# ClimeTrend/DMD-ERA5

Measured on AMD Instinct MI355X. Metric: rank-r SVD GB/s on ERA5 snapshot matrix (X resident in HBM), higher is better.
Workload: dtype f32; 1 GPU; cfg2: 1038240x8760 fp32 synthetic low-rank(64)+noise, row-centred, rank-50 method-of-snapshots SVD; m_per_gpu=1038240, m_total=1038240, n=8760, rank=50, svd_type=standard

## Files before the change

dmd_era5_amd/csrc/gemm_tn.hip:

```cpp
#include <stdarg.h>
#include <stdio.h>
#include <stdlib.h>

#include <algorithm>
#include <vector>

#include "dmdx_common.h"

thread_local unsigned long long* dmdx_clock_probe_ptr = nullptr;

int dmdx_device_cus() {
  static int cached[64] = {0};
  int dev = 0;
  if (hipGetDevice(&dev) != hipSuccess || dev < 0 || dev >= 64) return -1;
  if (cached[dev] == 0) {
    int v = 0;
    cached[dev] = (hipDeviceGetAttribute(&v, hipDeviceAttributeMultiprocessorCount, dev) == hipSuccess && v > 0) ? v : -1;
  }
  return cached[dev];
}

namespace {

constexpr int BT = 128;
constexpr int BK = 32;
constexpr int FOLD = 128;
constexpr int NTH = 256;

struct TnParams {
  const float* A;
  const float* B;
  int64_t lda, ldb;
  int64_t K;
  int nrow, ncol;
  int ntr, ntc;
  int ntiles;
  int syrk;
  int nsplit;
  int chunks_total;
  int chunks_per_split;
  double* P;
};

constexpr int MAXB = 16;
struct TnBatch {
  const float* A[MAXB];
  const float* B[MAXB];
  int64_t lda[MAXB];
  int64_t ldb[MAXB];
  int64_t K[MAXB];
  int chunks_total[MAXB];
  int chunks_per_split[MAXB];
  int nsplit[MAXB];
  int unit_begin[MAXB + 1];
  int slab_begin[MAXB + 1];
  int nblocks;
  unsigned long long* clk;
};

constexpr int SR = 8;
__device__ __host__ inline void decode_tri(int t, int nt, int& ta, int& tb) {
  int r0 = 0;
  for (;;) {
    int nrows = nt - r0 < SR ? nt - r0 : SR;
    int ncols = nt - r0;
    int cnt = nrows * (nrows + 1) / 2 + (ncols - nrows) * nrows;
    if (t < cnt) break;
    t -= cnt;
    r0 += SR;
  }
  int nrows = nt - r0 < SR ? nt - r0 : SR;
  int head = nrows * (nrows + 1) / 2;
  if (t < head) {
    int c = 0;
    while (t >= c + 1) { t -= c + 1; ++c; }
    tb = r0 + c;
    ta = r0 + t;
  } else {
    t -= head;
    tb = r0 + nrows + t / nrows;
    ta = r0 + t % nrows;
  }
}

__device__ inline void decode_tile(int syrk, int ntr, int ntc, int t, int& ta, int& tb) {
  if (syrk) {
    decode_tri(t, ntr, ta, tb);
  } else {
    int per_sr = SR * ntc;
    int sr = t / per_sr;
    int r0 = sr * SR;
    int nrows = ntr - r0 < SR ? ntr - r0 : SR;
    int tt = t - sr * per_sr;
    tb = tt / nrows;
    ta = r0 + tt % nrows;
  }
}

__device__ __forceinline__ int swz(int col) { return (col >> 1) & 7; }

__device__ inline f32x4 load4_tail(const float* p, int64_t k, int64_t kend) {
  f32x4 v = {0.f, 0.f, 0.f, 0.f};
#pragma unroll
  for (int e = 0; e < 4; ++e)
    if (k + e < kend) v[e] = p[e];
  return v;
}

#ifdef DMDX_STAMPS
__device__ unsigned long long dmdx_stamp[12];
#define DMDX_STAMP(var)                                                        \
  do {                                                                         \
    __builtin_amdgcn_sched_barrier(0);                                         \
    asm volatile("s_memtime %0\n\ts_waitcnt lgkmcnt(0)" : "=s"(var)::"memory"); \
    __builtin_amdgcn_sched_barrier(0);                                         \
  } while (0)
#else
#define DMDX_STAMP(var) do { } while (0)
#endif

#define DMDX_LDS_PTR(p) ((__attribute__((address_space(3))) void*)(p))
#define DMDX_GLB_PTR(p) ((const __attribute__((address_space(1))) void*)(p))

template <bool DMA, int ABL, int SK, int H16 = 0>
__device__ __forceinline__ void tn_unit(const TnParams& p, const int split, const int row0, const int col0,
                                        double* Pt, float* lds) {
  static_assert(!H16 || SK >= 1, "a 16-row block only below at least one 32-row block");
#ifdef DMDX_STAMPS
  unsigned long long pt0;
  asm volatile("s_memtime %0\n\ts_waitcnt lgkmcnt(0)" : "=s"(pt0)::"memory");
#endif
  constexpr int TM = SK ? 32 * SK + 16 * H16 : BT;
  constexpr int MI = SK ? SK : 2;
  constexpr int NI = SK ? 1 : 2;
  constexpr int NPA = (TM + 31) / 32;
  constexpr int NPIECE = TM / 8;
  constexpr int OPA = TM * BK, OPB = BT * BK, STG = OPA + OPB;

  const int c_begin = split * p.chunks_per_split;
  int c_end = c_begin + p.chunks_per_split;
  if (c_end > p.chunks_total) c_end = p.chunks_total;
  const int nchunks = c_end - c_begin;
  const int64_t kend = p.K;
  const int tail_chunk = (kend % BK) ? p.chunks_total - 1 : -1;

  const int tid = threadIdx.x;
  const int lane = tid & 63;
  const int wave = __builtin_amdgcn_readfirstlane(tid >> 6);
  const int wr = SK ? 0 : wave >> 1, wc = SK ? wave : wave & 1;
  const int l31 = lane & 31, lh = lane >> 5;

  const int ra0 = row0 < p.nrow ? row0 : p.nrow - 1;
  const int cb0 = col0 < p.ncol ? col0 : p.ncol - 1;
  const float* Abase = p.A + (int64_t)ra0 * p.lda;
  const float* Bbase = p.B + (int64_t)cb0 * p.ldb;
  unsigned aoff[NPA], boff[4];
  int stsa[NPA], stsb[4];
  int kqa[NPA], kqb[4];
#pragma unroll
  for (int i = 0; i < 4; ++i) {
    const int lc = DMA ? 32 * wave + 8 * i + (lane >> 3) : (tid >> 3) + 32 * i;
    const int q = DMA ? ((lane & 7) ^ swz(lc)) : (tid & 7);
    int cb = col0 + lc;
    cb = cb < p.ncol ? cb : p.ncol - 1;
    boff[i] = (unsigned)((int64_t)(cb - cb0) * p.ldb + 4 * q);
    stsb[i] = lc * BK + 4 * (DMA ? (lane & 7) : ((tid & 7) ^ swz(lc)));
    kqb[i] = 4 * q;
  }
#pragma unroll
  for (int i = 0; i < NPA; ++i) {
    const int lc = DMA ? (H16 ? 8 * (wave + 4 * i) : (TM / 4) * wave + 8 * i) + (lane >> 3) : (tid >> 3) + 32 * i;
    const int q = DMA ? ((lane & 7) ^ swz(lc)) : (tid & 7);
    int ca = row0 + (lc < TM ? lc : TM - 1);
    ca = ca < p.nrow ? ca : p.nrow - 1;
    aoff[i] = (unsigned)((int64_t)(ca - ra0) * p.lda + 4 * q);
    stsa[i] = lc * BK + 4 * (DMA ? (lane & 7) : ((tid & 7) ^ swz(lc)));
    kqa[i] = 4 * q;
  }

  const char* Adma = reinterpret_cast<const char*>(Abase) - (H16 ? 0 : 3072);
  const char* Bdma = reinterpret_cast<const char*>(Bbase) - 3072;
  unsigned aoffb[NPA], boffb[4];
#pragma unroll
  for (int i = 0; i < 4; ++i) boffb[i] = 4u * boff[i] + 3072u - 1024u * i;
#pragma unroll
  for (int i = 0; i < NPA; ++i) aoffb[i] = H16 ? 4u * aoff[i] : 4u * aoff[i] + 3072u - 1024u * i;

  f32x16 acc[MI][NI];
#pragma unroll
  for (int mi = 0; mi < MI; ++mi)
#pragma unroll
    for (int ni = 0; ni < NI; ++ni)
#pragma unroll
      for (int r = 0; r < 16; ++r) acc[mi][ni][r] = 0.f;

  f32x16 acc2[MI][NI];
#pragma unroll
  for (int mi = 0; mi < MI; ++mi)
#pragma unroll
    for (int ni = 0; ni < NI; ++ni)
#pragma unroll
      for (int r = 0; r < 16; ++r) acc2[mi][ni][r] = 0.f;
  f32x4 acch[2] = {{0.f, 0.f, 0.f, 0.f}, {0.f, 0.f, 0.f, 0.f}}, acch2[2] = {{0.f, 0.f, 0.f, 0.f}, {0.f, 0.f, 0.f, 0.f}};
  const int l15 = lane & 15, lkk = lane >> 4;
  const int lane_off = (64 * wr + 4 * lh) * BT + (SK ? 32 : 64) * wc + l31;
#define DMDX_BLOCK_OFF(mi, ni, r) ((32 * (mi) + ((r) & 3) + 8 * ((r) >> 2)) * BT + 32 * (ni))
#define DMDX_FOLD(mi, ni)                                                         \
  do {                                                                            \
    acc2[mi][ni] += acc[mi][ni];                                                  \
    _Pragma("unroll") for (int r = 0; r < 16; ++r) acc[mi][ni][r] = 0.f;          \
  } while (0)
#define DMDX_COMMIT(mi, ni)                                                       \
  do {                                                                            \
    double* q_ = Pt + lane_off;                                                   \
    _Pragma("unroll") for (int r = 0; r < 16; ++r)                                \
        __builtin_nontemporal_store((double)(acc[mi][ni][r] + acc2[mi][ni][r]),   \
                                    q_ + DMDX_BLOCK_OFF(mi, ni, r));              \
  } while (0)
#define DMDX_COMMIT_H16()                                                         \
  do {                                                                            \
    _Pragma("unroll") for (int hh = 0; hh < 2; ++hh)                              \
        _Pragma("unroll") for (int r = 0; r < 4; ++r)                             \
            __builtin_nontemporal_store((double)(acch[hh][r] + acch2[hh][r]),     \
                                        Pt + (32 * SK + 4 * lkk + r) * BT + 32 * wc + 16 * hh + l15); \
  } while (0)
#define DMDX_COMMIT_ALL()                                                         \
  do {                                                                            \
    if constexpr (H16 != 0) DMDX_COMMIT_H16();                                    \
    DMDX_COMMIT(0, 0);                                                            \
    if constexpr (MI >= 2) DMDX_COMMIT(MI >= 2 ? 1 : 0, 0);                       \
    if constexpr (NI == 2) {                                                      \
      DMDX_COMMIT(0, NI - 1);                                                     \
      DMDX_COMMIT(1, NI - 1);                                                     \
    }                                                                             \
    if constexpr (MI == 3) DMDX_COMMIT(MI - 1, 0);                                \
  } while (0)

  if (nchunks <= 0) {
    DMDX_COMMIT_ALL();
    return;
  }

  auto stage_regs = [&](int chunk, int st, bool tail) {
    const int64_t k0 = (int64_t)chunk * BK;
    f32x4 ra[NPA], rb[4];
#pragma unroll
    for (int i = 0; i < 4; ++i) {
      const float* pb = Bbase + k0 + boff[i];
      rb[i] = tail ? load4_tail(pb, k0 + kqb[i], kend) : f32x4{pb[0], pb[1], pb[2], pb[3]};
    }
#pragma unroll
    for (int i = 0; i < NPA; ++i) {
      const float* pa = Abase + k0 + aoff[i];
      ra[i] = tail ? load4_tail(pa, k0 + kqa[i], kend) : f32x4{pa[0], pa[1], pa[2], pa[3]};
    }
    const bool a_last_ok = !H16 || (DMA ? wave + 4 * (NPA - 1) < NPIECE : (tid >> 3) + 32 * (NPA - 1) < TM);
    float* as = lds + st * STG;
    float* bs = lds + st * STG + OPA;
#pragma unroll
    for (int i = 0; i < 4; ++i) *reinterpret_cast<f32x4*>(bs + stsb[i]) = rb[i];
#pragma unroll
    for (int i = 0; i < NPA; ++i)
      if (i + 1 < NPA || a_last_ok) *reinterpret_cast<f32x4*>(as + stsa[i]) = ra[i];
  };
#define DMDX_DMA_OP4(ptr, la, o0, o1, o2, o3)                                                      \
  asm volatile("s_mov_b32 m0, %[la_]\n\ts_nop 0\n\t"                                               \
               "global_load_lds_dwordx4 %[a0], %[ap_]\n\t"                                         \
               "global_load_lds_dwordx4 %[a1], %[ap_] offset:1024\n\t"                             \
               "global_load_lds_dwordx4 %[a2], %[ap_] offset:2048\n\t"                             \
               "global_load_lds_dwordx4 %[a3], %[ap_] offset:3072"                                 \
               :: [la_] "s"(la), [ap_] "s"(ptr), [a0] "v"(o0), [a1] "v"(o1), [a2] "v"(o2), [a3] "v"(o3) \
               : "memory")
#define DMDX_DMA_OP3(ptr, la, o0, o1, o2)                                                          \
  asm volatile("s_mov_b32 m0, %[la_]\n\ts_nop 0\n\t"                                               \
               "global_load_lds_dwordx4 %[a0], %[ap_]\n\t"                                         \
               "global_load_lds_dwordx4 %[a1], %[ap_] offset:1024\n\t"                             \
               "global_load_lds_dwordx4 %[a2], %[ap_] offset:2048"                                 \
               :: [la_] "s"(la), [ap_] "s"(ptr), [a0] "v"(o0), [a1] "v"(o1), [a2] "v"(o2)           \
               : "memory")
#define DMDX_DMA_OP1(ptr, la, o0)                                                                  \
  asm volatile("s_mov_b32 m0, %[la_]\n\ts_nop 0\n\t"                                               \
               "global_load_lds_dwordx4 %[a0], %[ap_]"                                             \
               :: [la_] "s"(la), [ap_] "s"(ptr), [a0] "v"(o0)                                       \
               : "memory")
#define DMDX_DMA_OP2(ptr, la, o0, o1)                                                              \
  asm volatile("s_mov_b32 m0, %[la_]\n\ts_nop 0\n\t"                                               \
               "global_load_lds_dwordx4 %[a0], %[ap_]\n\t"                                         \
               "global_load_lds_dwordx4 %[a1], %[ap_] offset:1024"                                 \
               :: [la_] "s"(la), [ap_] "s"(ptr), [a0] "v"(o0), [a1] "v"(o1)                         \
               : "memory")
#define DMDX_DMA_A(ap, la)                                                                         \
  do {                                                                                             \
    if constexpr (H16 != 0) {                                                                      \
      _Pragma("unroll") for (int i_ = 0; i_ < NPA; ++i_)                                           \
          if (i_ + 1 < NPA || wave + 4 * (NPA - 1) < NPIECE) DMDX_DMA_OP1(ap, (la) + 4096u * i_, aoffb[i_]); \
    } else if constexpr (NPA == 4) DMDX_DMA_OP4(ap, la, aoffb[0], aoffb[1], aoffb[NPA - 2], aoffb[NPA - 1]); \
    else if constexpr (NPA == 3) DMDX_DMA_OP3(ap, la, aoffb[0], aoffb[1], aoffb[NPA - 1]);         \
    else if constexpr (NPA == 2) DMDX_DMA_OP2(ap, la, aoffb[0], aoffb[NPA - 1]);                   \
    else DMDX_DMA_OP1(ap, la, aoffb[0]);                                                           \
  } while (0)
#define DMDX_DMA_B(bp, lb) DMDX_DMA_OP4(bp, lb, boffb[0], boffb[1], boffb[2], boffb[3])
#define DMDX_DMA_NEXT(ap, bp, la, lb) \
  do {                                \
    DMDX_DMA_A(ap, la);               \
    DMDX_DMA_B(bp, lb);               \
  } while (0)
  auto stage_dma = [&](int chunk, int st) {
    const int64_t k0 = (int64_t)chunk * BK;
    float* as = lds + st * STG + (H16 ? 8 * wave : (TM / 4) * wave) * BK;
    float* bs = lds + st * STG + OPA + (32 * wave) * BK;
    DMDX_DMA_NEXT(Adma + 4 * k0, Bdma + 4 * k0, (unsigned)(uintptr_t)DMDX_LDS_PTR(as),
                  (unsigned)(uintptr_t)DMDX_LDS_PTR(bs));
  };
  auto stage = [&](int chunk, int st) {
    if (DMA) {
      if (chunk != tail_chunk) stage_dma(chunk, st);
      else stage_regs(chunk, st, true);
    } else {
      stage_regs(chunk, st, chunk == tail_chunk);
    }
  };

  f32x4 fa0[MI], fb0[NI], fa1[MI], fb1[NI];
  f32x4 hA[2] = {{0.f, 0.f, 0.f, 0.f}, {0.f, 0.f, 0.f, 0.f}};
  f32x4 hB[2][2] = {{{0.f, 0.f, 0.f, 0.f}, {0.f, 0.f, 0.f, 0.f}}, {{0.f, 0.f, 0.f, 0.f}, {0.f, 0.f, 0.f, 0.f}}};
  int foff[4], foffh[2];
#pragma unroll
  for (int t = 0; t < 4; ++t) {
    foff[t] = l31 * BK + 4 * ((2 * t + lh) ^ swz(l31));
    if (t < 2) foffh[t] = l15 * BK + 4 * ((4 * t + lkk) ^ swz(l15));
  }
  const int frag_a = 64 * wr * BK, frag_b = (SK ? 32 : 64) * wc * BK;
#define DMDX_READ_FRAGS(FA, FB, st, t)                                               \
  do {                                                                               \
    if constexpr (H16 != 0) {                                                        \
      if constexpr ((t) % 2 == 0) {                                                  \
        const float* ah_ = lds + (st) * STG + 32 * SK * BK + foffh[(t) / 2];         \
        const float* bh_ = lds + (st) * STG + OPA + frag_b + foffh[(t) / 2];         \
        hA[(t) / 2] = *reinterpret_cast<const f32x4*>(ah_);                          \
        hB[(t) / 2][0] = *reinterpret_cast<const f32x4*>(bh_);                       \
        hB[(t) / 2][1] = *reinterpret_cast<const f32x4*>(bh_ + 16 * BK);             \
      }                                                                              \
    }                                                                                \
    const float* as_ = lds + (st) * STG + frag_a + foff[t];                          \
    const float* bs_ = lds + (st) * STG + OPA + frag_b + foff[t];                    \
    FA[0] = *reinterpret_cast<const f32x4*>(as_);                                    \
    if constexpr (MI >= 2) FA[MI >= 2 ? 1 : 0] = *reinterpret_cast<const f32x4*>(as_ + 32 * BK); \
    if constexpr (MI == 3) FA[MI - 1] = *reinterpret_cast<const f32x4*>(as_ + 64 * BK); \
    FB[0] = *reinterpret_cast<const f32x4*>(bs_);                                    \
    if constexpr (NI == 2) FB[NI - 1] = *reinterpret_cast<const f32x4*>(bs_ + 32 * BK); \
  } while (0)

  stage(c_begin, 0);
  if (nchunks > 1 && !(ABL & 1)) stage(c_begin + 1, 1);
  if (DMA) __builtin_amdgcn_s_waitcnt(0x0f70);
  __syncthreads();
  DMDX_READ_FRAGS(fa0, fb0, 0, 0);

#define DMDX_MFMA4(FA, FB, j)                                                                   \
  do {                                                                                          \
    _Pragma("unroll") for (int mi_ = 0; mi_ < MI; ++mi_)                                        \
        _Pragma("unroll") for (int ni_ = 0; ni_ < NI; ++ni_) acc[mi_][ni_] =                    \
            __builtin_amdgcn_mfma_f32_32x32x2f32(FA[mi_][j], FB[ni_][j], acc[mi_][ni_], 0, 0, 0); \
  } while (0)
#define DMDX_KSTEP(FA, FB, i)                                      \
  do {                                                             \
    DMDX_MFMA4(FA, FB, 0);                                         \
    DMDX_MFMA4(FA, FB, 1);                                         \
    DMDX_MFMA4(FA, FB, 2);                                         \
    DMDX_MFMA4(FA, FB, 3);                                         \
    if constexpr (H16 != 0) {                                      \
      _Pragma("unroll") for (int s_ = 0; s_ < 2; ++s_)             \
          _Pragma("unroll") for (int hh_ = 0; hh_ < 2; ++hh_) acch[hh_] = \
              __builtin_amdgcn_mfma_f32_16x16x4f32(hA[(i) / 2][2 * ((i) % 2) + s_], hB[(i) / 2][hh_][2 * ((i) % 2) + s_], acch[hh_], 0, 0, 0); \
    }                                                              \
    __builtin_amdgcn_sched_group_barrier(0x008, 4 * MI * NI + 4 * H16, 0);   \
  } while (0)

#ifdef DMDX_STAMPS
  unsigned long long rt0, rt1, ct0;
  asm volatile("s_memrealtime %0\n\ts_memtime %1\n\ts_waitcnt lgkmcnt(0)" : "=s"(rt0), "=s"(ct0)::"memory");
  unsigned long long st0 = 0, st1 = 0, st2 = 0, st2b = 0, st3 = 0, st4 = 0, sa0 = 0, sa1 = 0, sa2 = 0, sa3 = 0, sa5 = 0;
#endif
  int cur = 0;
  for (int c = 0; c < nchunks; ++c) {
    DMDX_STAMP(st0);
    const bool has_next = (c + 1 < nchunks) && !(ABL & 1);
    const int phase = c & (FOLD / 4 - 1), fq = (c / (FOLD / 4)) & 3;
    DMDX_STAMP(st1);
    DMDX_READ_FRAGS(fa1, fb1, cur, 1);
    __builtin_amdgcn_sched_group_barrier(0x100, MI + NI, 0);
    DMDX_KSTEP(fa0, fb0, 0);
    DMDX_READ_FRAGS(fa0, fb0, cur, 2);
    __builtin_amdgcn_sched_group_barrier(0x100, MI + NI + 3 * H16, 0);
    DMDX_KSTEP(fa1, fb1, 1);
    DMDX_READ_FRAGS(fa1, fb1, cur, 3);
    __builtin_amdgcn_sched_group_barrier(0x100, MI + NI, 0);
    DMDX_KSTEP(fa0, fb0, 2);
    DMDX_STAMP(st2);

    if (DMA) __builtin_amdgcn_s_waitcnt(0x0f70);
    DMDX_STAMP(st2b);
    if (!(ABL & 2)) __syncthreads();
    if (c + 2 < nchunks && !(ABL & 1)) stage(c_begin + c + 2, cur);
    cur ^= 1;
    DMDX_STAMP(st3);
    if (has_next) DMDX_READ_FRAGS(fa0, fb0, cur, 0);
    __builtin_amdgcn_sched_group_barrier(0x100, MI + NI + 3 * H16, 0);
    DMDX_KSTEP(fa1, fb1, 3);
    if (!(ABL & 8) && phase == FOLD / 4 - 1) {
      switch (fq) {
        case 0: DMDX_FOLD(0, 0); break;
        case 1:
          if constexpr (NI == 2) { DMDX_FOLD(0, NI - 1); }
          else if constexpr (MI == 3) { DMDX_FOLD(MI - 1, 0); }
          break;
        case 2: if constexpr (MI >= 2) { DMDX_FOLD(MI >= 2 ? 1 : 0, 0); } break;
        default:
          if constexpr (NI == 2) { DMDX_FOLD(1, NI - 1); }
          if constexpr (H16 != 0) {
#pragma unroll
            for (int hh = 0; hh < 2; ++hh) {
              acch2[hh] += acch[hh];
              acch[hh] = f32x4{0.f, 0.f, 0.f, 0.f};
            }
          }
          break;
      }
    }
#ifdef DMDX_STAMPS
    DMDX_STAMP(st4);
    sa0 += st1 - st0; sa1 += st2 - st1; sa2 += st3 - st2b; sa3 += st4 - st3; sa5 += st2b - st2;
#endif
  }
#ifdef DMDX_STAMPS
  if (lane == 0) {
    atomicAdd(&dmdx_stamp[0], sa0); atomicAdd(&dmdx_stamp[1], sa1);
    atomicAdd(&dmdx_stamp[2], sa2); atomicAdd(&dmdx_stamp[3], sa3);
    atomicAdd(&dmdx_stamp[5], sa5);
    asm volatile("s_memrealtime %0\n\ts_waitcnt lgkmcnt(0)" : "=s"(rt1)::"memory");
    atomicAdd(&dmdx_stamp[6], st4 - ct0);
    atomicAdd(&dmdx_stamp[7], rt1 - rt0);
    atomicAdd(&dmdx_stamp[4], (unsigned long long)nchunks);
    atomicAdd(&dmdx_stamp[8], ct0 - pt0);
    atomicAdd(&dmdx_stamp[10], 1ull);
  }
#endif
  DMDX_COMMIT_ALL();
#ifdef DMDX_STAMPS
  {
    unsigned long long et1;
    asm volatile("s_waitcnt vmcnt(0)\n\ts_memtime %0\n\ts_waitcnt lgkmcnt(0)" : "=s"(et1)::"memory");
    if (lane == 0) atomicAdd(&dmdx_stamp[9], et1 - st4);
  }
#endif
#undef DMDX_READ_FRAGS
#undef DMDX_MFMA4
#undef DMDX_KSTEP
#undef DMDX_DMA_NEXT
#undef DMDX_DMA_A
#undef DMDX_DMA_B
#undef DMDX_DMA_OP4
#undef DMDX_DMA_OP2
#undef DMDX_DMA_OP1
#undef DMDX_DMA_OP3
#undef DMDX_FOLD
#undef DMDX_COMMIT_ALL
#undef DMDX_COMMIT_H16
#undef DMDX_COMMIT
#undef DMDX_BLOCK_OFF
}

__device__ __forceinline__ int xcd_unit(int b, int total) {
  const int g = b >> 9;
  return ((g << 9) + 512 <= total) ? (g << 9) + (b & 7) * 64 + ((b & 511) >> 3) : b;
}

#ifndef DMDX_TN_ABL
#define DMDX_TN_ABL 0
#endif

template <bool DMA, int SK = 0, int H16 = 0>
__global__ __launch_bounds__(NTH, 2) void syrk_batch_kernel(TnParams p, TnBatch bt) {
  constexpr int TM = SK ? 32 * SK + 16 * H16 : BT;
  __shared__ __attribute__((aligned(16))) float lds[2 * (TM + BT) * BK];
  const int b = blockIdx.x;
  int j = 0;
  while (j + 1 < bt.nblocks && b >= bt.unit_begin[j + 1]) ++j;
  const int total = bt.nsplit[j] * p.ntiles;
  const int local = b - bt.unit_begin[j];
  if (local >= total) return;
  const int pos = xcd_unit(local, total);
  const int split = pos / p.ntiles;
  const int tile = pos - split * p.ntiles;
  int ta, tb;
  decode_tile(p.syrk, p.ntr, p.ntc, tile, ta, tb);
  p.A = bt.A[j];
  p.B = bt.B[j];
  p.lda = bt.lda[j];
  p.ldb = bt.ldb[j];
  p.K = bt.K[j];
  p.chunks_total = bt.chunks_total[j];
  p.chunks_per_split = bt.chunks_per_split[j];
  double* Pt = p.P + ((size_t)(bt.slab_begin[j] + split) * p.ntiles + tile) * (TM * BT);
  unsigned long long c0 = 0, r0 = 0;
  if (bt.clk != nullptr) {
    c0 = __builtin_amdgcn_s_memtime();
    r0 = __builtin_amdgcn_s_memrealtime();
  }
  tn_unit<DMA, DMDX_TN_ABL, SK, H16>(p, split, ta * TM, tb * BT, Pt, lds);
  if (bt.clk != nullptr) {
    const unsigned long long c1 = __builtin_amdgcn_s_memtime(), r1 = __builtin_amdgcn_s_memrealtime();
    if (threadIdx.x == 0) {
      atomicAdd(&bt.clk[0], c1 - c0);
      atomicAdd(&bt.clk[1], r1 - r0);
      atomicAdd(&bt.clk[2], 1ull);
    }
  }
}

__global__ __launch_bounds__(256) void gemm_tn_reduce_kernel(
    const double* P, int nsplit, int ntiles, int ntr, int ntc, int syrk, int nrow, int ncol,
    double* D64, int64_t ld64, float* D32, int64_t ld32, int accumulate, int tm) {
  __shared__ double tr[32][33];
  const int nsb = ((tm + 31) / 32) * 4;
  const int tile = blockIdx.x / nsb;
  const int sb = blockIdx.x - tile * nsb;
  const int tile_elems = tm * BT;
  int ta, tb;
  decode_tile(syrk, ntr, ntc, tile, ta, tb);
  const int row0 = ta * tm, col0 = tb * BT;
  const int tx = threadIdx.x & 31, ty = threadIdx.x >> 5;
  const bool diag = syrk && (ta == tb);
  const int si = (sb >> 2) * 32, sj = (sb & 3) * 32;
  if (diag && si > sj) return;
  if (row0 + si >= nrow || col0 + sj >= ncol) return;
  double v[4] = {0.0, 0.0, 0.0, 0.0};
  const double* src = P + (size_t)tile * tile_elems + (si + ty) * BT + sj + tx;
  for (int sp = 0; sp < nsplit; ++sp) {
    const double* q = src + (size_t)sp * ntiles * tile_elems;
#pragma unroll
    for (int k = 0; k < 4; ++k)
      if (si + ty + 8 * k < tm) v[k] += q[8 * k * BT];
  }
#pragma unroll
  for (int k = 0; k < 4; ++k) {
    const int i = si + ty + 8 * k, j = sj + tx;
    const int gi = row0 + i, gj = col0 + j;
    const bool keep = !(diag && i > j) && i < tm;
    if (keep && gi < nrow && gj < ncol) {
      double o = v[k];
      if (accumulate) o += D64[(int64_t)gi * ld64 + gj];
      D64[(int64_t)gi * ld64 + gj] = o;
      if (D32) D32[(int64_t)gi * ld32 + gj] = (float)o;
    }
    tr[ty + 8 * k][tx] = v[k];
  }
  if (syrk) {
    __syncthreads();
#pragma unroll
    for (int k = 0; k < 4; ++k) {
      const int i = si + tx, j = sj + ty + 8 * k;
      const double s = tr[tx][ty + 8 * k];
      const int gi = row0 + i, gj = col0 + j;
      const bool keep = !(diag && i >= j) && i < tm;
      if (keep && gi < nrow && gj < ncol) {
        double o = s;
        if (accumulate) o += D64[(int64_t)gj * ld64 + gi];
        D64[(int64_t)gj * ld64 + gi] = o;
        if (D32) D32[(int64_t)gj * ld32 + gi] = (float)o;
      }
    }
  }
}

struct Plan {
  int tm;
  int syrk;
  int ntr, ntc, ntiles, nsplit, chunks_total, chunks_per_split;
};

int64_t fit_last_round(int64_t chunks, int64_t units_per_split, int64_t want, int64_t hi) {
  if (getenv("DMDX_TN_NO_TAILFIT") != nullptr) return want;
  auto fill = [&](int64_t w) {
    const int64_t cps = (chunks + w - 1) / w;
    const int64_t ns = cps > 0 ? (chunks + cps - 1) / cps : 0;
    const double r = (double)(units_per_split * ns) / 512.0;
    return r > 0.0 ? r / (double)(int64_t)(r + 0.999999) : 1.0;
  };
  int64_t best = want;
  double bf = fill(want);
  if (bf < 0.92)
    for (int64_t w = want + 1; bf < 0.97 && w <= hi; ++w)
      if (fill(w) > bf) { bf = fill(w); best = w; }
  return best;
}

Plan make_plan(int64_t K, int64_t nrow, int64_t ncol, int syrk, int share = 1) {
  Plan pl;
  pl.tm = BT;
  const int gram = syrk;
  if (syrk && nrow <= 96) syrk = 0;
  pl.syrk = syrk;
  if (!syrk) {
    int64_t best = (nrow + BT - 1) / BT * BT;
    for (int tm : {112, 96, 80, 64, 48, 32}) {
      if (gram && tm % 32) continue;
      const int64_t padded = (nrow + tm - 1) / tm * tm;
      if (padded < best && (tm > 48 || nrow <= tm)) { best = padded; pl.tm = tm; }
    }
  }
  if (const char* e = getenv("DMDX_TN_FORCE_TM")) {
    const int f = atoi(e);
    if (!syrk && f >= 32 && f <= 128 && f % 16 == 0 && (f > 48 || nrow <= f)) pl.tm = f;
  }
  pl.ntr = (int)((nrow + pl.tm - 1) / pl.tm);
  pl.ntc = (int)((ncol + BT - 1) / BT);
  pl.ntiles = syrk ? pl.ntr * (pl.ntr + 1) / 2 : pl.ntr * pl.ntc;
  pl.chunks_total = (int)((K + BK - 1) / BK);
  if (pl.chunks_total < 1) pl.chunks_total = 1;
  int64_t max_cps = 2048;
  if (const char* e = getenv("DMDX_TN_MAX_CPS")) max_cps = atoll(e) > 0 ? atoll(e) : max_cps;
  int64_t rounds = gram ? (pl.ntiles >= 64 ? 20 : 2) : 6;
  if (const char* e = getenv("DMDX_TN_ROUNDS")) rounds = atoll(e) > 0 ? atoll(e) : rounds;
  const int64_t per_split = (int64_t)pl.ntiles * share;
  int64_t want = (rounds * 512 + per_split - 1) / per_split;
  int64_t by_len = (pl.chunks_total + max_cps - 1) / max_cps;
  if (want < by_len) want = by_len;
  int64_t maxs = pl.chunks_total / 8;
  if (maxs < 1) maxs = 1;
  if (want > maxs) want = maxs;
  if (want < 1) want = 1;
  if (want > 256) want = 256;
  want = fit_last_round(pl.chunks_total, per_split, want, std::min({maxs, (int64_t)256, 2 * want + 2}));
  pl.chunks_per_split = (int)((pl.chunks_total + want - 1) / want);
  pl.nsplit = (pl.chunks_total + pl.chunks_per_split - 1) / pl.chunks_per_split;
  return pl;
}

inline int group_len(int nblocks, int j0) { return std::min(nblocks - j0, MAXB); }

size_t batch_ws(const int64_t* K, int nblocks, int64_t nrow, int64_t ncol, int syrk) {
  size_t need = 0;
  for (int j0 = 0; j0 < nblocks; j0 += MAXB) {
    const int nb = group_len(nblocks, j0);
    size_t slabs = 0;
    Plan pl{};
    for (int j = 0; j < nb; ++j) {
      pl = make_plan(K[j0 + j], nrow, ncol, syrk, nb);
      slabs += (size_t)pl.nsplit;
    }
    need = std::max(need, slabs * (size_t)pl.ntiles * pl.tm * BT * sizeof(double));
  }
  return need;
}

int run_batch(const float* const* A, const int64_t* lda, const float* const* B, const int64_t* ldb,
              const int64_t* K, int nblocks, int64_t nrow, int64_t ncol, int syrk, double* D64, int64_t ld64,
              float* D32, int64_t ld32, int accumulate, void* ws, hipStream_t stream, bool probe) {
  for (int j0 = 0; j0 < nblocks; j0 += MAXB) {
    const int nb = group_len(nblocks, j0);
    TnBatch bt{};
    TnParams p{};
    bool aligned = true;
    int units = 0, slabs = 0;
    Plan pl{};
    for (int j = 0; j < nb; ++j) {
      const int64_t la = lda[j0 + j], lb = ldb[j0 + j];
      pl = make_plan(K[j0 + j], nrow, ncol, syrk, nb);
      bt.A[j] = A[j0 + j];
      bt.B[j] = B[j0 + j];
      bt.lda[j] = la;
      bt.ldb[j] = lb;
      bt.K[j] = K[j0 + j];
      bt.chunks_total[j] = pl.chunks_total;
      bt.chunks_per_split[j] = pl.chunks_per_split;
      bt.nsplit[j] = pl.nsplit;
      bt.unit_begin[j] = units;
      bt.slab_begin[j] = slabs;
      const int u = pl.nsplit * pl.ntiles;
      units += (j + 1 < nb) ? (u + 511) / 512 * 512 : u;
      slabs += pl.nsplit;
      aligned = aligned && (la % 4 == 0) && (lb % 4 == 0) && dmdx_aligned16(A[j0 + j]) &&
                dmdx_aligned16(B[j0 + j]) && la < (int64_t(1) << 22) && lb < (int64_t(1) << 22);
    }
    bt.unit_begin[nb] = units;
    bt.slab_begin[nb] = slabs;
    bt.nblocks = nb;
    bt.clk = probe ? dmdx_clock_probe_ptr : nullptr;
    p.nrow = (int)nrow;
    p.ncol = (int)ncol;
    p.ntr = pl.ntr; p.ntc = pl.ntc; p.ntiles = pl.ntiles; p.syrk = pl.syrk;
    p.nsplit = slabs;
    p.P = reinterpret_cast<double*>(ws);
    const dim3 grid((unsigned)units);
    switch (pl.tm) {
#define DMDX_TN_CASE(TMV, SKV, HV)                                                                          \
      case TMV:                                                                                             \
        if (aligned) hipLaunchKernelGGL((syrk_batch_kernel<true, SKV, HV>), grid, dim3(NTH), 0, stream, p, bt);    \
        else hipLaunchKernelGGL((syrk_batch_kernel<false, SKV, HV>), grid, dim3(NTH), 0, stream, p, bt);    \
        break
      DMDX_TN_CASE(32, 1, 0); DMDX_TN_CASE(48, 1, 1); DMDX_TN_CASE(64, 2, 0); DMDX_TN_CASE(80, 2, 1);
      DMDX_TN_CASE(96, 3, 0); DMDX_TN_CASE(112, 3, 1); DMDX_TN_CASE(128, 0, 0);
#undef DMDX_TN_CASE
      default: dmdx_set_error("gemm_tn: no kernel for tile height %d", pl.tm); return DMDX_E_INVALID;
    }
    DMDX_LAUNCH_CHECK();
    hipLaunchKernelGGL(gemm_tn_reduce_kernel, dim3(pl.ntiles * ((pl.tm + 31) / 32) * 4), dim3(256), 0, stream, p.P, slabs,
                       pl.ntiles, pl.ntr, pl.ntc, pl.syrk, (int)nrow, (int)ncol, D64, ld64, D32, ld32,
                       (accumulate || j0 > 0) ? 1 : 0, pl.tm);
    DMDX_LAUNCH_CHECK();
  }
  return 0;
}

constexpr int XT = 128, XL = 32, XK = 64;
constexpr int XSTG = (XL + XT) * XK;
constexpr int XFOLD = 128;

struct XtyBatch {
  const float* X[MAXB];
  const float* Y[MAXB];
  int64_t ldx[MAXB], ldy[MAXB];
  int chunks[MAXB], cps[MAXB], nsplit[MAXB];
  int unit_begin[MAXB + 1];
  int nblocks, ntiles, na, nb;
  double* P;
};

__device__ __forceinline__ void xty_dma(unsigned lds_addr, unsigned off, const char* base) {
  asm volatile("s_mov_b32 m0, %0\n\ts_nop 0\n\tglobal_load_lds_dwordx4 %1, %2"
               :: "s"(lds_addr), "v"(off), "s"(base) : "memory");
}

template <int T4>
__global__ __launch_bounds__(NTH, 2) void xty_small_kernel(XtyBatch bt) {
  __shared__ __attribute__((aligned(16))) float lds[2 * XSTG];
  const int tid = threadIdx.x, lane = tid & 63;
  const int wave = __builtin_amdgcn_readfirstlane(tid >> 6);
  const int l31 = lane & 31, lh = lane >> 5;
  const int u = blockIdx.x;
  int j = 0;
  while (j + 1 < bt.nblocks && u >= bt.unit_begin[j + 1]) ++j;
  const int local = u - bt.unit_begin[j];
  const int split = local / bt.ntiles, tile = local - split * bt.ntiles;
  const int c_begin = split * bt.cps[j];
  int c_end = c_begin + bt.cps[j];
  if (c_end > bt.chunks[j]) c_end = bt.chunks[j];
  const int nch = c_end - c_begin;
  const int col0 = tile * XT;
  const int64_t ldx = bt.ldx[j], ldy = bt.ldy[j];
  const int cb0 = col0 < bt.na ? col0 : bt.na - 1;
  const char* Xb = reinterpret_cast<const char*>(bt.X[j] + (int64_t)cb0 * ldx) + (int64_t)c_begin * XK * 4;
  const char* Yb = reinterpret_cast<const char*>(bt.Y[j]) + (int64_t)c_begin * XK * 4;

  unsigned xoff[8], yoff[2];
#pragma unroll
  for (int i = 0; i < 8; ++i) {
    const int lc = 32 * wave + 4 * i + (lane >> 4);
    int cg = col0 + lc;
    cg = cg < bt.na ? cg : bt.na - 1;
    const int g = (lane & 15) ^ (lc & 15);
    xoff[i] = (unsigned)(((int64_t)(cg - cb0) * ldx + 4 * g) * 4);
  }
#pragma unroll
  for (int i = 0; i < 2; ++i) {
    const int lc = 8 * wave + 4 * i + (lane >> 4);
    const int cg = lc < bt.nb ? lc : bt.nb - 1;
    const int g = (lane & 15) ^ (lc & 15);
    yoff[i] = (unsigned)(((int64_t)cg * ldy + 4 * g) * 4);
  }
  auto issue = [&](int c, int st) {
    const char* xb = Xb + (int64_t)c * (XK * 4);
    const char* yb = Yb + (int64_t)c * (XK * 4);
    float* ys = lds + st * XSTG + (8 * wave) * XK;
    float* xs = lds + st * XSTG + XL * XK + (32 * wave) * XK;
#pragma unroll
    for (int i = 0; i < 2; ++i) xty_dma((unsigned)(uintptr_t)DMDX_LDS_PTR(ys + 4 * i * XK), yoff[i], yb);
#pragma unroll
    for (int i = 0; i < 8; ++i) xty_dma((unsigned)(uintptr_t)DMDX_LDS_PTR(xs + 4 * i * XK), xoff[i], xb);
  };

  if constexpr (T4 >= 0) {
    constexpr int NT = T4 > 0 ? T4 : 1;
    const int c15 = lane & 15, kk = lane >> 4;
    f32x4 a16[8], a16b[8], at[2][NT], atb[2][NT];
#pragma unroll
    for (int b = 0; b < 8; ++b) { a16[b] = f32x4{0.f, 0.f, 0.f, 0.f}; a16b[b] = f32x4{0.f, 0.f, 0.f, 0.f}; }
#pragma unroll
    for (int h = 0; h < 2; ++h)
#pragma unroll
      for (int q = 0; q < NT; ++q) { at[h][q] = f32x4{0.f, 0.f, 0.f, 0.f}; atb[h][q] = f32x4{0.f, 0.f, 0.f, 0.f}; }
    if (nch > 0) issue(0, 0);
    if (nch > 1) issue(1, 1);
    const int ko16 = 4 * ((4 * wave + kk) ^ c15);
    for (int c = 0; c < nch; ++c) {
      const int st = c & 1;
      if (c + 1 < nch) asm volatile("s_waitcnt vmcnt(10)" ::: "memory");
      else asm volatile("s_waitcnt vmcnt(0)" ::: "memory");
      __syncthreads();
      const float* ys = lds + st * XSTG;
      const float* xs = ys + XL * XK;
      const f32x4 fa = *reinterpret_cast<const f32x4*>(ys + c15 * XK + ko16);
      f32x4 fb[8];
#pragma unroll
      for (int b = 0; b < 8; ++b) fb[b] = *reinterpret_cast<const f32x4*>(xs + (16 * b + c15) * XK + ko16);
#pragma unroll
      for (int e = 0; e < 4; ++e)
#pragma unroll
        for (int b = 0; b < 8; ++b) a16[b] = __builtin_amdgcn_mfma_f32_16x16x4f32(fa[e], fb[b][e], a16[b], 0, 0, 0);
      if constexpr (T4 > 0) {
#pragma unroll
        for (int p4 = 0; p4 < 4; ++p4) {
          f32x4 ax[2], by[NT];
#pragma unroll
          for (int h = 0; h < 2; ++h)
            ax[h] = *reinterpret_cast<const f32x4*>(xs + (64 * h + lane) * XK + 4 * ((4 * wave + p4) ^ (lane & 15)));
#pragma unroll
          for (int q = 0; q < NT; ++q) {
            const int yc = 16 + 4 * q + (lane & 3);
            by[q] = *reinterpret_cast<const f32x4*>(ys + yc * XK + 4 * ((4 * wave + p4) ^ (yc & 15)));
          }
#pragma unroll
          for (int e = 0; e < 4; ++e)
#pragma unroll
            for (int h = 0; h < 2; ++h)
#pragma unroll
              for (int q = 0; q < NT; ++q) at[h][q] = __builtin_amdgcn_mfma_f32_4x4x1f32(ax[h][e], by[q][e], at[h][q], 0, 0, 0);
        }
      }
      __syncthreads();
      if (c + 2 < nch) issue(c + 2, st);
      if ((c & (XFOLD - 1)) == XFOLD - 1) {
#pragma unroll
        for (int b = 0; b < 8; ++b) { a16b[b] += a16[b]; a16[b] = f32x4{0.f, 0.f, 0.f, 0.f}; }
#pragma unroll
        for (int h = 0; h < 2; ++h)
#pragma unroll
          for (int q = 0; q < NT; ++q) { atb[h][q] += at[h][q]; at[h][q] = f32x4{0.f, 0.f, 0.f, 0.f}; }
      }
    }
    float* red = lds + wave * (XL * XT);
#pragma unroll
    for (int b = 0; b < 8; ++b)
#pragma unroll
      for (int r = 0; r < 4; ++r) red[(4 * kk + r) * XT + 16 * b + c15] = a16[b][r] + a16b[b][r];
    for (int o = 4 * lane; o < 16 * XT; o += 256)
      *reinterpret_cast<f32x4*>(red + 16 * XT + o) = f32x4{0.f, 0.f, 0.f, 0.f};
// ... 337 lines not shown
```

Baseline: 61.18 GB/s.

## Compute SYRK k-step with three-way bf16 split MFMA instead of fp32 path

Adds a plane-split path for the 128x128 SYRK tile. Each fp32 operand is split into high, mid and low bf16 planes, and six bf16 32x32x16 MFMA products replace the fp32 MFMA. NaN/Inf inputs are detected with a ballot and the planes are sanitised from LDS. DMA offsets are parked in extra LDS to relieve register pressure. The path is on by default unless DMDX_K1_ARITH=f32 is set. The aim is to use the higher bf16 matrix throughput on MI355X while keeping near-fp32 accuracy, at the cost of extra split ALU work, more MFMA issues and extra LDS.

```diff
diff --git a/dmd_era5_amd/csrc/bf16_split.h b/dmd_era5_amd/csrc/bf16_split.h
--- /dev/null
+++ b/dmd_era5_amd/csrc/bf16_split.h
@@ -0,0 +1,91 @@
+#pragma once
+#include <math.h>
+#include <stdint.h>
+#include <string.h>
+
+#if defined(__HIPCC__) || defined(__CUDACC__)
+#define DMDX_SPLIT_HD __host__ __device__ inline
+#else
+#define DMDX_SPLIT_HD inline
+#endif
+
+namespace bf16split {
+
+constexpr uint32_t TOP16 = 0xFFFF0000u;
+
+DMDX_SPLIT_HD uint32_t bits(float x) {
+  uint32_t u;
+  __builtin_memcpy(&u, &x, 4);
+  return u;
+}
+DMDX_SPLIT_HD float from_bits(uint32_t u) {
+  float x;
+  __builtin_memcpy(&x, &u, 4);
+  return x;
+}
+
+DMDX_SPLIT_HD uint32_t pack2(uint32_t a, uint32_t b) {
+#if defined(__HIP_DEVICE_COMPILE__)
+  return __builtin_amdgcn_perm(b, a, 0x07060302u);
+#else
+  return (b & TOP16) | (a >> 16);
+#endif
+}
+
+DMDX_SPLIT_HD float detect(float x, float s) { return __builtin_fmaf(x, 0.0f, s); }
+DMDX_SPLIT_HD bool fired(float s) { return s != s; }
+
+DMDX_SPLIT_HD bool non_finite(uint32_t u) { return (u & 0x7F800000u) == 0x7F800000u; }
+
+DMDX_SPLIT_HD void split1(float x, uint32_t& h, uint32_t& m, uint32_t& l) {
+  h = bits(x) & TOP16;
+  const float r = x - from_bits(h);
+  m = bits(r) & TOP16;
+  l = bits(r - from_bits(m));
+}
+
+DMDX_SPLIT_HD void split2_fast(float x0, float x1, uint32_t& H, uint32_t& M, uint32_t& L) {
+  uint32_t h0, m0, l0, h1, m1, l1;
+  split1(x0, h0, m0, l0);
+  split1(x1, h1, m1, l1);
+  H = pack2(bits(x0), bits(x1));
+  M = pack2(m0, m1);
+  L = pack2(l0, l1);
+}
+
+#if defined(__HIPCC__)
+typedef float f32x2_t __attribute__((ext_vector_type(2)));
+typedef uint32_t u32x2_t __attribute__((ext_vector_type(2)));
+DMDX_SPLIT_HD void split2_fast_pair(f32x2_t x, uint32_t& H, uint32_t& M, uint32_t& L) {
+  const u32x2_t xb = __builtin_bit_cast(u32x2_t, x);
+  const f32x2_t r = x - __builtin_bit_cast(f32x2_t, xb & TOP16);
+  const u32x2_t mb = __builtin_bit_cast(u32x2_t, r) & TOP16;
+  const u32x2_t lb = __builtin_bit_cast(u32x2_t, r - __builtin_bit_cast(f32x2_t, mb));
+  H = pack2(xb[0], xb[1]);
+  M = pack2(mb[0], mb[1]);
+  L = pack2(lb[0], lb[1]);
+}
+DMDX_SPLIT_HD f32x2_t detect_pair(f32x2_t x, f32x2_t s) { return __builtin_elementwise_fma(x, (f32x2_t){0.0f, 0.0f}, s); }
+#endif
+
+DMDX_SPLIT_HD uint32_t non_finite_halves(uint32_t P) {
+  const uint32_t t = ((P & 0x7F807F80u) + 0x00800080u) & 0x80008000u;
+  return (t >> 15) * 0xFFFFu;
+}
+
+DMDX_SPLIT_HD void make_safe2(float x0, float x1, uint32_t& H, uint32_t& M, uint32_t& L) {
+  H |= (x0 != x0 ? 0x00000040u : 0u) | (x1 != x1 ? 0x00400000u : 0u);
+  const uint32_t keep = ~non_finite_halves(H);
+  M &= keep;
+  L &= keep;
+}
+
+DMDX_SPLIT_HD uint32_t sanitise2(uint32_t H) { return H & ~non_finite_halves(H); }
+
+DMDX_SPLIT_HD void split2_safe(float x0, float x1, uint32_t& H, uint32_t& HP, uint32_t& M, uint32_t& L) {
+  split2_fast(x0, x1, H, M, L);
+  make_safe2(x0, x1, H, M, L);
+  HP = sanitise2(H);
+}
+
+}
diff --git a/dmd_era5_amd/csrc/gemm_tn.hip b/dmd_era5_amd/csrc/gemm_tn.hip
--- a/dmd_era5_amd/csrc/gemm_tn.hip
+++ b/dmd_era5_amd/csrc/gemm_tn.hip
@@ -5,6 +5,7 @@
 #include <algorithm>
 #include <vector>
 
+#include "bf16_split.h"
 #include "dmdx_common.h"
 
 thread_local unsigned long long* dmdx_clock_probe_ptr = nullptr;
@@ -26,6 +27,8 @@
 constexpr int BK = 32;
 constexpr int FOLD = 128;
 constexpr int NTH = 256;
+typedef __bf16 bf16x8 __attribute__((ext_vector_type(8)));
+typedef unsigned u32x4 __attribute__((ext_vector_type(4)));
 
 struct TnParams {
   const float* A;
@@ -119,13 +122,20 @@
 #define DMDX_STAMP(var) do { } while (0)
 #endif
 
+__device__ __forceinline__ int lane_now() {
+  unsigned z = 0u;
+  asm volatile("" : "+v"(z));
+  return (int)__builtin_amdgcn_mbcnt_hi(~0u, __builtin_amdgcn_mbcnt_lo(~0u, z));
+}
+
 #define DMDX_LDS_PTR(p) ((__attribute__((address_space(3))) void*)(p))
 #define DMDX_GLB_PTR(p) ((const __attribute__((address_space(1))) void*)(p))
 
-template <bool DMA, int ABL, int SK, int H16 = 0>
+template <bool DMA, int ABL, int SK, int H16 = 0, int PL = 0>
 __device__ __forceinline__ void tn_unit(const TnParams& p, const int split, const int row0, const int col0,
                                         double* Pt, float* lds) {
   static_assert(!H16 || SK >= 1, "a 16-row block only below at least one 32-row block");
+  static_assert(!PL || (SK == 0 && H16 == 0), "the plane k-step is built for the 128 x 128 tile only");
 #ifdef DMDX_STAMPS
   unsigned long long pt0;
   asm volatile("s_memtime %0\n\ts_waitcnt lgkmcnt(0)" : "=s"(pt0)::"memory");
@@ -204,6 +214,8 @@
   f32x4 acch[2] = {{0.f, 0.f, 0.f, 0.f}, {0.f, 0.f, 0.f, 0.f}}, acch2[2] = {{0.f, 0.f, 0.f, 0.f}, {0.f, 0.f, 0.f, 0.f}};
   const int l15 = lane & 15, lkk = lane >> 4;
   const int lane_off = (64 * wr + 4 * lh) * BT + (SK ? 32 : 64) * wc + l31;
+  auto lane_off_of = [&](int ln) { return (64 * wr + 4 * (ln >> 5)) * BT + (SK ? 32 : 64) * wc + (ln & 31); };
+  int lane_off_c = PL ? 0 : lane_off;
 #define DMDX_BLOCK_OFF(mi, ni, r) ((32 * (mi) + ((r) & 3) + 8 * ((r) >> 2)) * BT + 32 * (ni))
 #define DMDX_FOLD(mi, ni)                                                         \
   do {                                                                            \
@@ -212,7 +224,7 @@
   } while (0)
 #define DMDX_COMMIT(mi, ni)                                                       \
   do {                                                                            \
-    double* q_ = Pt + lane_off;                                                   \
+    double* q_ = Pt + lane_off_c;                                                 \
     _Pragma("unroll") for (int r = 0; r < 16; ++r)                                \
         __builtin_nontemporal_store((double)(acc[mi][ni][r] + acc2[mi][ni][r]),   \
                                     q_ + DMDX_BLOCK_OFF(mi, ni, r));              \
@@ -237,31 +249,65 @@
   } while (0)
 
   if (nchunks <= 0) {
+    if constexpr (PL != 0) lane_off_c = lane_off_of(lane_now());
     DMDX_COMMIT_ALL();
     return;
   }
 
-  auto stage_regs = [&](int chunk, int st, bool tail) {
+  auto stage_regs = [&](int chunk, int st, bool tail, const unsigned (&aoffb)[NPA], const unsigned (&boffb)[4]) {
     const int64_t k0 = (int64_t)chunk * BK;
     f32x4 ra[NPA], rb[4];
+    unsigned boff_[4], aoff_[NPA];
+    int stsb_[4], kqb_[4], stsa_[NPA], kqa_[NPA];
+    int tid_ = tid;
+    if constexpr (PL != 0) tid_ = 64 * wave + lane_now();
+    const int lane_ = tid_ & 63;
 #pragma unroll
     for (int i = 0; i < 4; ++i) {
-      const float* pb = Bbase + k0 + boff[i];
-      rb[i] = tail ? load4_tail(pb, k0 + kqb[i], kend) : f32x4{pb[0], pb[1], pb[2], pb[3]};
+      if constexpr (PL != 0 && DMA) {
+        const int lcb = 32 * wave + 8 * i + (lane_ >> 3), lca = (TM / 4) * wave + 8 * i + (lane_ >> 3);
+        kqb_[i] = 4 * ((lane_ & 7) ^ swz(lcb));
+        kqa_[i] = 4 * ((lane_ & 7) ^ swz(lca));
+        stsb_[i] = lcb * BK + 4 * (lane_ & 7);
+        stsa_[i] = lca * BK + 4 * (lane_ & 7);
+        boff_[i] = (boffb[i] - 3072u + 1024u * i) >> 2;
+        aoff_[i] = (aoffb[i] - 3072u + 1024u * i) >> 2;
+        asm volatile("" : "+v"(boff_[i]), "+v"(aoff_[i]));
+      } else if constexpr (PL != 0) {
+        const int lc = (tid_ >> 3) + 32 * i, q = tid_ & 7;
+        int cb = col0 + lc, ca = row0 + lc;
+        cb = cb < p.ncol ? cb : p.ncol - 1;
+        ca = ca < p.nrow ? ca : p.nrow - 1;
+        boff_[i] = (unsigned)((int64_t)(cb - cb0) * p.ldb + 4 * q);
+        aoff_[i] = (unsigned)((int64_t)(ca - ra0) * p.lda + 4 * q);
+        stsb_[i] = stsa_[i] = lc * BK + 4 * (q ^ swz(lc));
+        kqb_[i] = kqa_[i] = 4 * q;
+      } else {
+        boff_[i] = boff[i]; stsb_[i] = stsb[i]; kqb_[i] = kqb[i];
+        if (i < NPA) {
+          const int ia = i < NPA ? i : 0;
+          aoff_[ia] = aoff[ia]; stsa_[ia] = stsa[ia]; kqa_[ia] = kqa[ia];
+        }
+      }
+    }
+#pragma unroll
+    for (int i = 0; i < 4; ++i) {
+      const float* pb = Bbase + k0 + boff_[i];
+      rb[i] = tail ? load4_tail(pb, k0 + kqb_[i], kend) : f32x4{pb[0], pb[1], pb[2], pb[3]};
     }
 #pragma unroll
     for (int i = 0; i < NPA; ++i) {
-      const float* pa = Abase + k0 + aoff[i];
-      ra[i] = tail ? load4_tail(pa, k0 + kqa[i], kend) : f32x4{pa[0], pa[1], pa[2], pa[3]};
+      const float* pa = Abase + k0 + aoff_[i];
+      ra[i] = tail ? load4_tail(pa, k0 + kqa_[i], kend) : f32x4{pa[0], pa[1], pa[2], pa[3]};
     }
     const bool a_last_ok = !H16 || (DMA ? wave + 4 * (NPA - 1) < NPIECE : (tid >> 3) + 32 * (NPA - 1) < TM);
     float* as = lds + st * STG;
     float* bs = lds + st * STG + OPA;
 #pragma unroll
-    for (int i = 0; i < 4; ++i) *reinterpret_cast<f32x4*>(bs + stsb[i]) = rb[i];
+    for (int i = 0; i < 4; ++i) *reinterpret_cast<f32x4*>(bs + stsb_[i]) = rb[i];
 #pragma unroll
     for (int i = 0; i < NPA; ++i)
-      if (i + 1 < NPA || a_last_ok) *reinterpret_cast<f32x4*>(as + stsa[i]) = ra[i];
+      if (i + 1 < NPA || a_last_ok) *reinterpret_cast<f32x4*>(as + stsa_[i]) = ra[i];
   };
 #define DMDX_DMA_OP4(ptr, la, o0, o1, o2, o3)                                                      \
   asm volatile("s_mov_b32 m0, %[la_]\n\ts_nop 0\n\t"                                               \
@@ -305,21 +351,22 @@
     DMDX_DMA_A(ap, la);               \
     DMDX_DMA_B(bp, lb);               \
   } while (0)
-  auto stage_dma = [&](int chunk, int st) {
+  auto stage_dma = [&](int chunk, int st, const unsigned (&aoffb)[NPA], const unsigned (&boffb)[4]) {
     const int64_t k0 = (int64_t)chunk * BK;
     float* as = lds + st * STG + (H16 ? 8 * wave : (TM / 4) * wave) * BK;
     float* bs = lds + st * STG + OPA + (32 * wave) * BK;
-    DMDX_DMA_NEXT(Adma + 4 * k0, Bdma + 4 * k0, (unsigned)(uintptr_t)DMDX_LDS_PTR(as),
-                  (unsigned)(uintptr_t)DMDX_LDS_PTR(bs));
+    DMDX_DMA_NEXT(Adma + 4 * k0, Bdma + 4 * k0, __builtin_amdgcn_readfirstlane((unsigned)(uintptr_t)DMDX_LDS_PTR(as)),
+                  __builtin_amdgcn_readfirstlane((unsigned)(uintptr_t)DMDX_LDS_PTR(bs)));
   };
-  auto stage = [&](int chunk, int st) {
+  auto stage_with = [&](int chunk, int st, const unsigned (&ao)[NPA], const unsigned (&bo)[4]) {
     if (DMA) {
-      if (chunk != tail_chunk) stage_dma(chunk, st);
-      else stage_regs(chunk, st, true);
+      if (chunk != tail_chunk) stage_dma(chunk, st, ao, bo);
+      else stage_regs(chunk, st, true, ao, bo);
     } else {
-      stage_regs(chunk, st, chunk == tail_chunk);
+      stage_regs(chunk, st, chunk == tail_chunk, ao, bo);
     }
   };
+  auto stage = [&](int chunk, int st) { stage_with(chunk, st, aoffb, boffb); };
 
   f32x4 fa0[MI], fb0[NI], fa1[MI], fb1[NI];
   f32x4 hA[2] = {{0.f, 0.f, 0.f, 0.f}, {0.f, 0.f, 0.f, 0.f}};
@@ -383,6 +430,135 @@
   unsigned long long st0 = 0, st1 = 0, st2 = 0, st2b = 0, st3 = 0, st4 = 0, sa0 = 0, sa1 = 0, sa2 = 0, sa3 = 0, sa5 = 0;
 #endif
   int cur = 0;
+  if constexpr (PL != 0) {
+    unsigned PH[4][4], PM[4][4], PLo[4][4];
+#define DMDX_SPLIT_GROUP(g)                                                                      \
+  do {                                                                                           \
+    __builtin_amdgcn_sched_barrier(0);   \
+    bf16split::f32x2_t d_ = {0.f, 0.f};                                                          \
+    _Pragma("unroll") for (int b_ = 0; b_ < 4; ++b_) {                                           \
+      const f32x4 e_ = b_ < 2 ? fa0[b_ & 1] : fb0[b_ & 1], o_ = b_ < 2 ? fa1[b_ & 1] : fb1[b_ & 1]; \
+      _Pragma("unroll") for (int q_ = 0; q_ < 4; ++q_) {                                         \
+        const bf16split::f32x2_t x_ = q_ < 2 ? bf16split::f32x2_t{e_[2 * (q_ & 1)], e_[2 * (q_ & 1) + 1]} \
+                                             : bf16split::f32x2_t{o_[2 * (q_ & 1)], o_[2 * (q_ & 1) + 1]}; \
+        unsigned h_, m_, l_;                                                                     \
+        bf16split::split2_fast_pair(x_, h_, m_, l_);                                             \
+        PH[b_][q_] = h_; PM[b_][q_] = m_; PLo[b_][q_] = l_;                                      \
+        if (!(ABL & 16)) d_ = bf16split::detect_pair(x_, d_);                                    \
+      }                                                                                          \
+    }                                                                                            \
+    bad = !(ABL & 16) && __builtin_amdgcn_ballot_w64(__builtin_isunordered(d_[0], d_[1])) != 0ull;   \
+    if (bad) {   \
+       \
+      _Pragma("unroll") for (int b_ = 0; b_ < 4; ++b_) {                                         \
+        const float* s_ = lds + cur * STG + (b_ < 2 ? frag_a : OPA + frag_b) + (b_ & 1) * 32 * BK; \
+        __builtin_amdgcn_sched_barrier(0);                                                       \
+        int f0_ = foff[0];                                                                       \
+        asm volatile("" : "+v"(f0_));                    \
+        const f32x4 e_ = *reinterpret_cast<const f32x4*>(s_ + (f0_ ^ (8 * (2 * (g)))));          \
+        const f32x4 o_ = *reinterpret_cast<const f32x4*>(s_ + (f0_ ^ (8 * (2 * (g) + 1))));      \
+        _Pragma("unroll") for (int q_ = 0; q_ < 4; ++q_) {                                       \
+          const float x0_ = q_ < 2 ? e_[2 * (q_ & 1)] : o_[2 * (q_ & 1)];                        \
+          const float x1_ = q_ < 2 ? e_[2 * (q_ & 1) + 1] : o_[2 * (q_ & 1) + 1];                \
+          unsigned h_ = PH[b_][q_], m_ = PM[b_][q_], l_ = PLo[b_][q_];                           \
+          bf16split::make_safe2(x0_, x1_, h_, m_, l_);                                           \
+          PH[b_][q_] = h_; PM[b_][q_] = m_; PLo[b_][q_] = l_;                                    \
+        }                                                                                        \
+        __builtin_amdgcn_sched_barrier(0);                                                       \
+      }                                                                                          \
+    }                                                                                            \
+  } while (0)
+#define DMDX_PLANE(P, b) __builtin_bit_cast(bf16x8, (u32x4){P[b][0], P[b][1], P[b][2], P[b][3]})
+#define DMDX_MFMA_PL(PA, PB)                                                                     \
+  do {                                                                                           \
+    _Pragma("unroll") for (int mi_ = 0; mi_ < 2; ++mi_)                                          \
+        _Pragma("unroll") for (int ni_ = 0; ni_ < 2; ++ni_) acc[mi_][ni_] =                      \
+            __builtin_amdgcn_mfma_f32_32x32x16_bf16(DMDX_PLANE(PA, mi_), DMDX_PLANE(PB, 2 + ni_), acc[mi_][ni_], 0, 0, 0); \
+  } while (0)
+#define DMDX_GROUP_MFMA(rd, st, t0, fresh)                                                            \
+  do {                                                                                           \
+     \
+    int f0_ = foff[0];                                                                           \
+    asm volatile("" : "+v"(f0_));                                                                \
+    const int fe_ = f0_ ^ (8 * (t0)), fo_ = f0_ ^ (8 * ((t0) + 1));                              \
+    if (rd) {                                                                                    \
+      const float* as_ = lds + (st) * STG + frag_a;                                              \
+      fa0[0] = *reinterpret_cast<const f32x4*>(as_ + fe_);                                       \
+      fa0[1] = *reinterpret_cast<const f32x4*>(as_ + fe_ + 32 * BK);                             \
+      fa1[0] = *reinterpret_cast<const f32x4*>(as_ + fo_);                                       \
+      fa1[1] = *reinterpret_cast<const f32x4*>(as_ + fo_ + 32 * BK);                             \
+    }                                                                                            \
+    if (fresh) {   \
+      _Pragma("unroll") for (int mi_ = 0; mi_ < 2; ++mi_)                                        \
+          _Pragma("unroll") for (int ni_ = 0; ni_ < 2; ++ni_) acc[mi_][ni_] =                    \
+              __builtin_amdgcn_mfma_f32_32x32x16_bf16(DMDX_PLANE(PH, mi_), DMDX_PLANE(PH, 2 + ni_), f32x16(0.f), 0, 0, 0); \
+    } else {                                                                                     \
+      DMDX_MFMA_PL(PH, PH);                                                                      \
+    }                                                                                            \
+    if (bad) {                                                                                   \
+      _Pragma("unroll") for (int b_ = 0; b_ < 4; ++b_)                                           \
+          _Pragma("unroll") for (int q_ = 0; q_ < 4; ++q_) PH[b_][q_] = bf16split::sanitise2(PH[b_][q_]); \
+    }                                                                                            \
+    DMDX_MFMA_PL(PH, PLo);                                                                       \
+    DMDX_MFMA_PL(PLo, PH);                                                                       \
+    __builtin_amdgcn_sched_barrier(0);                                                           \
+    if (rd) {                                                                                    \
+      const float* bs_ = lds + (st) * STG + OPA + frag_b;                                        \
+      fb0[0] = *reinterpret_cast<const f32x4*>(bs_ + fe_);                                       \
+      fb0[1] = *reinterpret_cast<const f32x4*>(bs_ + fe_ + 32 * BK);                             \
+      fb1[0] = *reinterpret_cast<const f32x4*>(bs_ + fo_);                                       \
+      fb1[1] = *reinterpret_cast<const f32x4*>(bs_ + fo_ + 32 * BK);                             \
+    }                                                                                            \
+    DMDX_MFMA_PL(PH, PM);                                                                        \
+    DMDX_MFMA_PL(PM, PH);                                                                        \
+    DMDX_MFMA_PL(PM, PM);                                                                        \
+  } while (0)
+    bool bad = false;
+    DMDX_READ_FRAGS(fa1, fb1, 0, 1);
+    if constexpr (DMA) {
+      u32x4* park = reinterpret_cast<u32x4*>(lds + 2 * STG) + 2 * tid;
+      park[0] = u32x4{aoffb[0], aoffb[1], aoffb[2], aoffb[3]};
+      park[1] = u32x4{boffb[0], boffb[1], boffb[2], boffb[3]};
+    }
+    for (int c = 0; c < nchunks; ++c) {
+      DMDX_STAMP(st0);
+      const bool has_next = (c + 1 < nchunks) && !(ABL & 1);
+      DMDX_STAMP(st1);
+      DMDX_SPLIT_GROUP(0);
+      DMDX_GROUP_MFMA(true, cur, 2, true);
+      DMDX_SPLIT_GROUP(1);
+      DMDX_STAMP(st2);
+      unsigned pa[NPA] = {0u, 0u, 0u, 0u}, pb[4] = {0u, 0u, 0u, 0u};
+      if (DMA && c + 2 < nchunks) {
+        const u32x4* park = reinterpret_cast<const u32x4*>(lds + 2 * STG) + 2 * (64 * wave + lane_now());
+        const u32x4 a_ = park[0], b_ = park[1];
+        pa[0] = a_[0]; pa[1] = a_[1]; pa[2] = a_[2]; pa[3] = a_[3];
+        pb[0] = b_[0]; pb[1] = b_[1]; pb[2] = b_[2]; pb[3] = b_[3];
+      }
+
+      if (DMA) __builtin_amdgcn_s_waitcnt(0x0f70);
+      DMDX_STAMP(st2b);
+      if (!(ABL & 2)) __syncthreads();
+      if (c + 2 < nchunks && !(ABL & 1)) stage_with(c_begin + c + 2, cur, pa, pb);
+      cur ^= 1;
+      DMDX_STAMP(st3);
+      DMDX_GROUP_MFMA(has_next, cur, 0, false);
+      if (!(ABL & 8)) {
+        DMDX_FOLD(0, 0); DMDX_FOLD(0, NI - 1); DMDX_FOLD(MI - 1, 0); DMDX_FOLD(MI - 1, NI - 1);
+      }
+#ifdef DMDX_STAMPS
+      DMDX_STAMP(st4);
+      sa0 += st1 - st0; sa1 += st2 - st1; sa2 += st3 - st2b; sa3 += st4 - st3; sa5 += st2b - st2;
+#endif
+    }
+    {
+      lane_off_c = lane_off_of(lane_now());
+    }
+#undef DMDX_GROUP_MFMA
+#undef DMDX_MFMA_PL
+#undef DMDX_PLANE
+#undef DMDX_SPLIT_GROUP
+  } else {
   for (int c = 0; c < nchunks; ++c) {
     DMDX_STAMP(st0);
     const bool has_next = (c + 1 < nchunks) && !(ABL & 1);
@@ -433,6 +609,7 @@
     sa0 += st1 - st0; sa1 += st2 - st1; sa2 += st3 - st2b; sa3 += st4 - st3; sa5 += st2b - st2;
 #endif
   }
+  }
 #ifdef DMDX_STAMPS
   if (lane == 0) {
     atomicAdd(&dmdx_stamp[0], sa0); atomicAdd(&dmdx_stamp[1], sa1);
@@ -480,10 +657,10 @@
 #define DMDX_TN_ABL 0
 #endif
 
-template <bool DMA, int SK = 0, int H16 = 0>
+template <bool DMA, int SK = 0, int H16 = 0, int PL = 0>
 __global__ __launch_bounds__(NTH, 2) void syrk_batch_kernel(TnParams p, TnBatch bt) {
   constexpr int TM = SK ? 32 * SK + 16 * H16 : BT;
-  __shared__ __attribute__((aligned(16))) float lds[2 * (TM + BT) * BK];
+  __shared__ __attribute__((aligned(16))) float lds[2 * (TM + BT) * BK + (PL && DMA ? 8 * NTH : 0)];
   const int b = blockIdx.x;
   int j = 0;
   while (j + 1 < bt.nblocks && b >= bt.unit_begin[j + 1]) ++j;
@@ -504,14 +681,15 @@
   p.chunks_per_split = bt.chunks_per_split[j];
   double* Pt = p.P + ((size_t)(bt.slab_begin[j] + split) * p.ntiles + tile) * (TM * BT);
   unsigned long long c0 = 0, r0 = 0;
+  const int wave0 = __builtin_amdgcn_readfirstlane(threadIdx.x >> 6);
   if (bt.clk != nullptr) {
     c0 = __builtin_amdgcn_s_memtime();
     r0 = __builtin_amdgcn_s_memrealtime();
   }
-  tn_unit<DMA, DMDX_TN_ABL, SK, H16>(p, split, ta * TM, tb * BT, Pt, lds);
+  tn_unit<DMA, DMDX_TN_ABL, SK, H16, PL>(p, split, ta * TM, tb * BT, Pt, lds);
   if (bt.clk != nullptr) {
     const unsigned long long c1 = __builtin_amdgcn_s_memtime(), r1 = __builtin_amdgcn_s_memrealtime();
-    if (threadIdx.x == 0) {
+    if (wave0 == 0 && lane_now() == 0) {
       atomicAdd(&bt.clk[0], c1 - c0);
       atomicAdd(&bt.clk[1], r1 - r0);
       atomicAdd(&bt.clk[2], 1ull);
@@ -694,6 +872,11 @@
     p.nsplit = slabs;
     p.P = reinterpret_cast<double*>(ws);
     const dim3 grid((unsigned)units);
+    const char* arith = getenv("DMDX_K1_ARITH");
+    if (pl.tm == BT && pl.syrk && !(arith != nullptr && strcmp(arith, "f32") == 0)) {
+      if (aligned) hipLaunchKernelGGL((syrk_batch_kernel<true, 0, 0, 1>), grid, dim3(NTH), 0, stream, p, bt);
+      else hipLaunchKernelGGL((syrk_batch_kernel<false, 0, 0, 1>), grid, dim3(NTH), 0, stream, p, bt);
+    } else
     switch (pl.tm) {
 #define DMDX_TN_CASE(TMV, SKV, HV)                                                                          \
       case TMV:                                                                                             \
```

Result: faster. 66.38 GB/s (median of 6 runs) (+8.5%).
